# pixeru/bpm_analysis

Measured on AMD Instinct MI355X. Metric: audio-samples/sec (filter+envelope+peaks), 1024x60s@44.1kHz batch, 1 & 8 GPU, higher is better.
Workload: dtype f64; 1 GPU; 1024 x 60 s 44100 Hz mono int16 recordings per GPU, native mode (filter+envelope+noise floor+raw peaks); mode=native, parallelism=file-sharded x1, batch_pipeline=False

## Files before the change

bpm_analysis_amd/_native.py:

```python
from __future__ import annotations

import ctypes
import os

_HERE = os.path.dirname(os.path.abspath(__file__))
LIB_PATH = os.environ.get("BPMX_LIB") or os.path.join(_HERE, "libbpmx.so")

ABI_VERSION = 2

DT_U8, DT_I16, DT_I32, DT_F32, DT_F64 = 0, 1, 2, 3, 4
MODE_REFERENCE, MODE_NATIVE = 0, 1
STAGE_ENVELOPE, STAGE_FLOOR, STAGE_PEAKS, STAGE_ALL = 1, 2, 4, 7
F_STATIC_FLOOR, F_DRAFT_FLOOR, F_NAN_FLOOR, F_TOO_SHORT, F_BAD_WINDOW = 1, 2, 4, 8, 16
F_TROUGH_TIE, F_PEAK_TIE = 32, 64
F_TROUGH_ORDERED, F_PEAK_ORDERED = 128, 256
OPT_ROLLQ_MERGE = 1
OPT_NATIVE_F64 = 2
OPT_HILBERT_ROCFFT = 4
OPT_DRAFT_FULL = 8
OPT_ROLLQ_NOPRUNE = 16
OPT_DRAFT_GLOBAL_RANK = 32
OPT_ROLLQ_GLOBAL = 64
OPT_NATIVE_DMA = 128
OPT_PEAKS_GLOBAL = 256
OPT_HILBERT_R2C = 512
OPT_REF_SERIAL_MEAN = 1024
OPT_STATS = 2048
OPT_HILBERT_BLUESTEIN = 4096
OPT_REF_NOSPLIT = 8192
STAT_RAW_TROUGHS, STAT_UNDECIDED, STAT_FULL_DRAFT, NSTATS = 0, 1, 2, 8
OK, E_ARG, E_HIP, E_LIMIT, E_NODEV = 0, -1, -2, -3, -4

EXPORTS = ["bpmx_abi_version", "bpmx_last_error", "bpmx_create", "bpmx_destroy", "bpmx_decimated_length",
           "bpmx_run", "bpmx_run_ordered", "bpmx_synth", "bpmx_synth_host", "bpmx_profile", "bpmx_profile_read", "bpmx_profile_only",
           "bpmx_stats", "bpmx_set_pipeline"]


class Params(ctypes.Structure):
    _fields_ = [("mode", ctypes.c_int32), ("stages", ctypes.c_int32), ("dtype", ctypes.c_int32),
                ("channels", ctypes.c_int32), ("fs", ctypes.c_int32), ("ds", ctypes.c_int32),
                ("sr", ctypes.c_int32), ("env_window", ctypes.c_int32), ("distance", ctypes.c_int32),
                ("noise_window", ctypes.c_int32), ("min_periods", ctypes.c_int32), ("options", ctypes.c_int32),
                ("trough_prom_q", ctypes.c_double), ("peak_prom_q", ctypes.c_double),
                ("noise_floor_q", ctypes.c_double), ("fallback_q", ctypes.c_double),
                ("reject_mult", ctypes.c_double),
                ("ba_b", ctypes.c_double * 5), ("ba_a", ctypes.c_double * 5), ("ba_zi", ctypes.c_double * 4),
                ("sos", ctypes.c_double * 12), ("sos_zi", ctypes.c_double * 4)]


class Batch(ctypes.Structure):
    _fields_ = [("n_files", ctypes.c_int32), ("reserved", ctypes.c_int32), ("pcm", ctypes.c_void_p),
                ("frame_offsets", ctypes.POINTER(ctypes.c_int64))]


class Out(ctypes.Structure):
    _fields_ = [("env", ctypes.c_void_p), ("floor", ctypes.c_void_p), ("y", ctypes.c_void_p),
                ("troughs", ctypes.c_void_p), ("peaks", ctypes.c_void_p), ("n_troughs", ctypes.c_void_p),
                ("n_peaks", ctypes.c_void_p), ("flags", ctypes.c_void_p), ("n_raw_troughs", ctypes.c_void_p)]


class PeakOrder(ctypes.Structure):
    _fields_ = [("cand", ctypes.c_void_p * 2), ("n_cand", ctypes.c_void_p * 2),
                ("rank", ctypes.c_void_p * 2), ("use_rank", ctypes.c_void_p * 2)]


class BpmxError(RuntimeError):

    def __init__(self, msg: str = "", code: int = None):
        super().__init__(msg)
        self.code = code

    @property
    def per_file(self) -> bool:
        return self.code in (E_ARG, E_LIMIT)


class BpmxArgError(BpmxError, ValueError):
    """BPMX_E_ARG: an argument the reference's own calls reject with ValueError
    (scipy find_peaks' distance check, pandas' rolling-window checks); the
    message is the library's, which repeats the reference-side wording."""


_lib = None
# ... 51 lines not shown
```

bpm_analysis_amd/csrc/bpmx_api.hip:

```cpp
#include <hip/hip_runtime.h>

#include <algorithm>
#include <climits>
#include <cstdio>
#include <cstring>
#include <cstdlib>
#include <map>
#include <mutex>
#include <string>
#include <vector>

#include "bpmx_common.h"
#include "bpmx_kernels.h"
#include "bpmx_ctx.h"
#include "bpmx_native.h"
#include "bpmx_fpscan.h"
#include "bpmx_synth.h"

#include <rocprofiler-sdk-roctx/roctx.h>

using namespace bpmx;

namespace bpmx {
thread_local std::string g_err;
// ... 623 lines not shown
        }
        if (bad_window)
            LAUNCH(ctx, s, "k_flag_window", k_flag_window, dim3((F + 255) / 256), dim3(256), 0, s, F, d_run1,
                   (int32_t *)O->flags);
        const bool floor_wm = !(P->options & (BPMX_OPT_ROLLQ_MERGE | BPMX_OPT_ROLLQ_GLOBAL | BPMX_OPT_ROLLQ_NOPRUNE)) &&
                              maxnd <= WM_MMAX;
        if (noise_lazy && !floor_wm) {
            QuantArgs a;
            a.env = O->env; a.doff = d_doff; a.active = d_active; a.n_files = F; a.qv = qv; a.skip_le = QR_MAX;
            a.n_levels = 1; a.q[0] = P->noise_floor_q; a.slot[0] = 1 << Q_NOISE;
            a.skip = d_run1; a.stats = 0;
            LAUNCH(ctx, s, "k_quantile_reg", k_quantile_reg, dim3(F), dim3(QR_T), 0, s, a, bs);
        }
        const int64_t W = bad_window ? P->min_periods : P->noise_window;
        const int cap = (int)((W + RQ_T - 1 + 63) / 64 * 64);
        const size_t lds = rollq_lds_bytes(RQ_T, cap);
        const bool use_wm = !(P->options & (BPMX_OPT_ROLLQ_MERGE | BPMX_OPT_ROLLQ_GLOBAL));
        const bool need_merge = !use_wm || maxnd > WM_MMAX;
        const bool merge_g = need_merge && (cap > 32 * RQ_T || W + RQ_T >= 65000 || (P->options & BPMX_OPT_ROLLQ_GLOBAL));
        const int64_t gcap = (std::min<int64_t>(W + RQ_T, maxnd + 64) + 63) / 64 * 64;
        const size_t lds_g = rollq_g_lds_bytes(RQ_T, gcap);
        if (merge_g && lds_g > 160 * 1024)
            return fail(BPMX_E_LIMIT, "noise window and recording both longer than " +
                                          std::to_string((160 * 1024 - 16384) / 4 * 64) + " samples");
        uint16_t *wm_pos = use_wm ? (uint16_t *)ctx->buf("wm_pos", (size_t)sumnd * 2, &rc) : nullptr;
        int32_t *wm_full = use_wm ? (int32_t *)ctx->buf("wm_full", (size_t)F * 4, &rc) : nullptr;
        if (rc != BPMX_OK) return rc;
        const int64_t wm_n = std::min<int64_t>(maxnd, WM_MMAX);
        const size_t wm_lds_p = wm_layout(wm_n, true).total, wm_lds = wm_layout(wm_n, false).total;
        const int64_t wm_c = (WM_MMAX - W + 1) / 64 * 64;
        const bool wm_chunks = use_wm && maxnd > WM_MMAX && !(P->options & BPMX_OPT_ROLLQ_NOPRUNE) && wm_c >= 2048;
        const int64_t wm_nch = wm_chunks ? (maxnd + wm_c - 1) / wm_c : 1;
        int32_t *wm_fail = wm_chunks ? (int32_t *)ctx->buf("wm_fail", (size_t)F * 4, &rc) : nullptr;
        uint16_t *wm_pos_ch = wm_chunks ? (uint16_t *)ctx->buf("wm_pos_ch", (size_t)F * wm_nch * WM_PMAX * 2, &rc) : nullptr;
        if (rc != BPMX_OK) return rc;
        if (wm_nch > 65535) return fail(BPMX_E_LIMIT, "recording too long for the chunked rolling quantile");
        const dim3 g2((unsigned)std::min<int64_t>((maxnd + 255) / 256, std::max<int64_t>(8, 2048 / F)), F);
        auto interp = [&](const int32_t *run, const int64_t *tr, const int32_t *ntr, int64_t skip_gt) -> int {
            InterpArgs a;
            a.env = O->env; a.doff = d_doff; a.troughs = tr; a.ntr = ntr; a.run = run; a.n_files = F;
            a.dense = dense; a.skip_n = use_wm ? WM_MMAX : -1; a.skip_gt = skip_gt;
            const dim3 gi = maxnd <= WM_MMAX && use_wm ? dim3(2, (unsigned)F) : g2;
            LAUNCH(ctx, s, "k_interp", k_interp, gi, dim3(256), 0, s, a);
            return BPMX_OK;
        };
        auto rollq = [&](const int32_t *run, const int64_t *tr, const int32_t *ntr, double *outp,
                         int32_t *allnan, const double *tv) -> int {
            RollqArgs a;
            a.dense = dense; a.doff = d_doff; a.troughs = tr; a.tv = tv; a.run = run; a.n_files = F;
            a.env = O->env; a.ntr = ntr;
            a.window = (int32_t)W; a.min_periods = P->min_periods; a.cap = cap; a.q = P->noise_floor_q;
            a.out = outp; a.allnan = allnan; a.wm_max = use_wm ? WM_MMAX : 0;
            a.wm_chunk = 0; a.wm_fail = wm_fail; a.wm_pos_ch = wm_pos_ch;
            int rq_rc = BPMX_OK;
            int32_t *vfl = need_merge ? (int32_t *)ctx->buf("rollq_valid", (size_t)F * 8, &rq_rc) : nullptr;
            if (rq_rc != BPMX_OK) return rq_rc;
            a.vfirst = vfl;
            a.vlast = vfl ? vfl + F : nullptr;
            if (need_merge) {
                HIP_TRY(hipMemsetAsync(a.vfirst, 0x7F, (size_t)F * 4, s));
                HIP_TRY(hipMemsetAsync(a.vlast, 0xFF, (size_t)F * 4, s));
            }
            if (wm_chunks) {
                HIP_TRY(hipMemsetAsync(wm_fail, 0, (size_t)F * 4, s));
                a.wm_chunk = (int32_t)wm_c;
            }
            if (need_merge && (rq_rc = interp(run, tr, ntr, wm_chunks ? WM_MMAX : INT64_MAX)) != BPMX_OK) return rq_rc;
            if (use_wm) {
                wm_lds_attr(ctx->device);
                if (!(P->options & BPMX_OPT_ROLLQ_NOPRUNE))
                    LAUNCH(ctx, s, "k_rollq_wm", k_rollq_wm_t<true>, dim3(F, (unsigned)wm_nch), dim3(WM_T),
                           std::max(wm_lds_p, wm_lds), s, a, wm_pos, wm_full);
                else
                    LAUNCH(ctx, s, "k_rollq_wm[full]", k_rollq_wm_t<false>, dim3(F), dim3(WM_T), wm_lds, s, a, wm_pos,
                           wm_full);
            }
            if (!need_merge) return BPMX_OK;
            RollqArgs fill = a;
            if (wm_chunks) {
                a.run = wm_fail;
                if ((rq_rc = interp(wm_fail, tr, ntr, INT64_MAX)) != BPMX_OK) return rq_rc;
            }
            a.chunk = 8192;
            while (a.chunk > 1024 && (int64_t)F * ((maxnd + a.chunk - 1) / a.chunk) < 1024) a.chunk >>= 1;
            if (merge_g) a.chunk = std::max<int64_t>(a.chunk, (W + RQ_T - 1) / RQ_T * RQ_T);
            const int64_t nch = (maxnd + a.chunk - 1) / a.chunk;
            if (nch > 65535) return fail(BPMX_E_LIMIT, "recording too long for the chunked rolling quantile");
            const dim3 gq((unsigned)F, (unsigned)nch);
            if (merge_g) {
                a.gcap = gcap;
                a.gv = (double *)ctx->buf("rollq_gv", (size_t)F * nch * 2 * gcap * 8, &rq_rc);
                a.gp = (int32_t *)ctx->buf("rollq_gp", (size_t)F * nch * 2 * gcap * 4, &rq_rc);
                if (rq_rc != BPMX_OK) return rq_rc;
                (void)hipFuncSetAttribute((const void *)k_rolling_quantile_g<RQ_T>,
                                          hipFuncAttributeMaxDynamicSharedMemorySize, (int)lds_g);
                LAUNCH(ctx, s, "k_rolling_quantile", (k_rolling_quantile_g<RQ_T>), gq, dim3(RQ_T), lds_g, s, a);
            } else if (cap <= 16 * RQ_T) {
                (void)hipFuncSetAttribute((const void *)k_rolling_quantile<RQ_T, 16>,
                                          hipFuncAttributeMaxDynamicSharedMemorySize, (int)lds);
                LAUNCH(ctx, s, "k_rolling_quantile", (k_rolling_quantile<RQ_T, 16>), gq, dim3(RQ_T), lds, s, a);
            } else {
                (void)hipFuncSetAttribute((const void *)k_rolling_quantile<RQ_T, 32>,
                                          hipFuncAttributeMaxDynamicSharedMemorySize, (int)lds);
                LAUNCH(ctx, s, "k_rolling_quantile", (k_rolling_quantile<RQ_T, 32>), gq, dim3(RQ_T), lds, s, a);
            }
            LAUNCH(ctx, s, "k_rollq_fill", k_rollq_fill, dim3(4, (unsigned)F), dim3(256), 0, s, fill);
            return BPMX_OK;
        };
        uint8_t *tdec = nullptr;
        int32_t *d_exact = d_run1, *d_runfb = nullptr;
        if (bounds) {
            tdec = (uint8_t *)ctx->buf("trough_dec", (size_t)sumnd, &rc);
            if (rc != BPMX_OK) return rc;
            d_exact = draft_masks;
            d_runfb = draft_masks + F;
            DraftBoundArgs a;
            a.env = O->env; a.doff = d_doff; a.raw = rawt; a.rawv = rawv; a.nraw = d_nraw; a.run = d_run1;
            a.n_files = F;
            a.window = (int32_t)W; a.min_periods = P->min_periods; a.q = P->noise_floor_q; a.mult = P->reject_mult;
            a.dec = tdec; a.exact = d_exact;
            a.local_m = (P->options & BPMX_OPT_DRAFT_GLOBAL_RANK) ? INT_MAX : DB_LOCAL_M;
            a.stats = d_stats;
            if (rc != BPMX_OK) return rc;
            const int64_t trmax = maxnd / std::max<int64_t>(1, P->distance) + 1;
            const unsigned gy = (unsigned)std::max<int64_t>(1, (trmax + DB_T - 1) / DB_T);
            a.vfl = draft_vfl;
            a.nund = draft_vfl + 2 * F;
            LAUNCH(ctx, s, "k_draft_bounds", k_draft_bounds, dim3(F, gy), dim3(DB_T), 0, s, a);
#ifndef BPMX_DP_GY
#define BPMX_DP_GY 4
#endif
            const unsigned gp = (unsigned)std::max<int64_t>(1, std::min<int64_t>(BPMX_DP_GY, (trmax + DP_CHUNK - 1) / DP_CHUNK));
            LAUNCH(ctx, s, "k_draft_points", k_draft_points<1>, dim3(F, gp), dim3(DB_T), 0, s, a);
            LAUNCH(ctx, s, "k_draft_points[wide]", k_draft_points<4>, dim3(F, gp), dim3(DB_T), 0, s, a);
        }
        SanitizeArgs sa;
        sa.env = O->env; sa.draft = draft; sa.doff = d_doff; sa.active = d_active; sa.raw = rawt; sa.nraw = d_nraw;
        sa.rawv = rawv; sa.outv = trv;
        sa.n_files = F; sa.mult = P->reject_mult; sa.out = O->troughs; sa.nout = O->n_troughs; sa.flags = O->flags;
        sa.run2 = d_run2; sa.dec = tdec; sa.exact = d_exact; sa.run_fb = d_runfb;
        if (floor_wm) {
            FloorWmArgs a;
            a.rq.dense = dense; a.rq.doff = d_doff; a.rq.n_files = F; a.rq.env = O->env;
            a.rq.window = (int32_t)W; a.rq.min_periods = P->min_periods; a.rq.cap = cap; a.rq.q = P->noise_floor_q;
            a.rq.wm_max = WM_MMAX; a.rq.wm_chunk = 0; a.rq.wm_fail = nullptr; a.rq.wm_pos_ch = nullptr;
            a.rq.vfirst = a.rq.vlast = nullptr; a.rq.chunk = 0; a.rq.gv = nullptr; a.rq.gp = nullptr; a.rq.gcap = 0;
            a.rq.troughs = nullptr; a.rq.tv = nullptr; a.rq.ntr = nullptr; a.rq.run = nullptr; a.rq.out = nullptr;
            a.rq.allnan = nullptr;
#ifdef BPMX_STAMPS
            a.rq.stamps = nullptr;
#endif
            sa.run2 = nullptr; sa.run_fb = nullptr;
            a.sa = sa;
            a.exact = d_exact;
            a.qv = qv;
            a.qn = QuantArgs{};
            if (noise_lazy) {
                a.qn.env = O->env; a.qn.doff = d_doff; a.qn.active = d_active; a.qn.n_files = F; a.qn.qv = qv;
                a.qn.skip_le = QR_MAX; a.qn.n_levels = 1; a.qn.q[0] = P->noise_floor_q; a.qn.slot[0] = 1 << Q_NOISE;
                a.qn.skip = nullptr; a.qn.stats = 0;
            }
            a.floor = O->floor; a.draft = draft; a.an_draft = d_an1; a.an_final = d_an2; a.full = wm_full;
            if ((rc = rollq(d_exact, rawt, d_nraw, draft, d_an1, rawv)) != BPMX_OK) return rc;
            wm_lds_attr(ctx->device);
            LAUNCH(ctx, s, "k_floor_wm", k_floor_wm, dim3(F), dim3(WM_T), std::max(wm_lds_p, wm_lds), s, a);
        }
        if (!floor_wm && (rc = rollq(d_exact, rawt, d_nraw, draft, d_an1, rawv)) != BPMX_OK) return rc;
        if (!floor_wm) {
            SanitizeArgs a;
            a.env = O->env; a.draft = draft; a.doff = d_doff; a.active = d_active; a.raw = rawt; a.nraw = d_nraw;
            a.rawv = rawv; a.outv = trv;
            a.n_files = F; a.mult = P->reject_mult; a.out = O->troughs; a.nout = O->n_troughs; a.flags = O->flags;
            a.run2 = d_run2; a.dec = tdec; a.exact = d_exact; a.run_fb = d_runfb;
            LAUNCH(ctx, s, "k_sanitize", k_sanitize, dim3(F), dim3(256), 0, s, a);
        }
        if (!floor_wm && bounds && (rc = rollq(d_runfb, rawt, d_nraw, draft, d_an1, rawv)) != BPMX_OK) return rc;
        if (!floor_wm && (rc = rollq(d_run2, O->troughs, O->n_troughs, O->floor, d_an2, trv)) != BPMX_OK) return rc;
        if (!floor_wm) {
            FinalArgs a;
            a.draft = draft; a.doff = d_doff; a.active = d_active; a.qv = qv; a.allnan_draft = d_an1;
            a.allnan_final = d_an2; a.n_files = F; a.floor = O->floor; a.flags = O->flags;
#ifndef BPMX_FF_WIDE
            const dim3 gf(maxnd > 65536 ? g2.x : 1u, (unsigned)F);
#else
            const dim3 gf = g2;
#endif
            LAUNCH(ctx, s, "k_floor_final", k_floor_final, gf, dim3(256), 0, s, a);
        }
    }

    if (do_peaks) {
        StageRange range("bpmx:peaks");
        PeakArgs a;
        a.env = O->env; a.height = O->floor; a.doff = d_doff; a.boff = d_boff; a.active = d_active;
        a.bmax = bmax; a.bmin = bmin; a.qv = qv; a.qslot = Q_PEAK; a.n_files = F; a.distance = P->distance;
        a.sign = 1.0; a.cand = cand; a.state = state; a.out = O->peaks; a.nout = O->n_peaks;
        a.run_out = nullptr; a.run_min = 0; a.tie_bit = BPMX_F_PEAK_TIE;
        a.scan_ok = fp_scan; a.scan_cnt = fp_scan + F;
        set_order(a, 1);
        FIND_PEAKS(a, "peaks");
    }
// ... 161 lines not shown
```

bpm_analysis_amd/csrc/bpmx_kernels.h:

```cpp
#ifndef BPMX_KERNELS_H
#define BPMX_KERNELS_H

#include "bpmx_common.h"

namespace bpmx {

enum { Q_TROUGH = 0, Q_PEAK = 1, Q_NOISE = 2, Q_FALLBACK = 3, Q_SLOTS = 4 };

struct InitOutArgs {
    const int32_t *active;
    int32_t *flags, *ntr, *npk, *runs, *nraw;
    int32_t *z1;
    int32_t *z2;
    int32_t *z3;
    int32_t n_files;
};
__device__ __forceinline__ void init_out_one(const InitOutArgs &I, int f) {
    const int F = I.n_files;
    I.flags[f] = I.active[f] ? 0 : BPMX_F_TOO_SHORT;
    if (I.ntr) I.ntr[f] = 0;
    if (I.npk) I.npk[f] = 0;
    for (int k = 0; k < 5; ++k) I.runs[(int64_t)k * F + f] = 0;
    if (I.nraw) I.nraw[f] = 0;
    if (I.z1) I.z1[f] = 0;
// ... 159 lines not shown
    int32_t *mtot;
    int32_t *mp;
    double *mh;
    double *vv;
    double *b32h, *b32l, *b32r;
    double *b1kh, *b1kl, *b1kr;
    int32_t *dfail;
    int32_t dchunk;
};
constexpr int FPC_T = 256, FPC_S = 1024, FPC_H = 1024, FPC_R = (FPC_S + FPC_H) / FPC_T;
__host__ __device__ inline int64_t fpl_b32_off(int64_t d0, int f) { return (d0 >> 5) + 4 * (int64_t)f; }
__host__ __device__ inline int64_t fpl_b1k_off(int64_t d0, int f) { return (d0 >> 10) + 4 * (int64_t)f; }
__global__ void k_fpl_scan(PeakArgs A, FplArgs L);
__global__ void k_fpl_place(PeakArgs A, FplArgs L);
__global__ void k_fpl_fill(PeakArgs A, FplArgs L);
__global__ void k_fpl_distance(PeakArgs A, FplArgs L);
__global__ void k_fpl_dist_ch(PeakArgs A, FplArgs L);
__global__ void k_fpl_prom(PeakArgs A, FplArgs L);
__global__ void k_fpl_compact(PeakArgs A, FplArgs L);

struct InterpArgs {
    const double *env;
    const int64_t *doff;
    const int64_t *troughs;
    const int32_t *ntr;
    const int32_t *run;
    int32_t n_files;
    double *dense;
    int64_t skip_n;
    int64_t skip_gt;
};

struct RollqArgs {
    const double *dense;
    const int64_t *doff;
    const int64_t *troughs;
    const int32_t *run;
    int32_t n_files, window, min_periods, cap;
    double q;
    double *out;
    int32_t *allnan;
    int32_t wm_max;
    const double *env;
    const double *tv;
    const int32_t *ntr;
    int64_t chunk;
    int32_t *vfirst, *vlast;
    double *gv;
    int32_t *gp;
    int64_t gcap;
    int32_t wm_chunk;
    int32_t *wm_fail;
    uint16_t *wm_pos_ch;
#ifdef BPMX_STAMPS
    unsigned long long *stamps;
#endif
};

struct SanitizeArgs {
    const double *env, *draft;
    const int64_t *doff;
    const int32_t *active;
    const int64_t *raw;
    const double *rawv;
    const int32_t *nraw;
    int32_t n_files;
    double mult;
    double *outv;
    int64_t *out;
    int32_t *nout;
    int32_t *flags;
    int32_t *run2;
    const uint8_t *dec;
    const int32_t *exact;
    int32_t *run_fb;
};

template <int NT>
__device__ __forceinline__ int sanitize_wg(const SanitizeArgs &A, int f, int *sh) {
    const int64_t d0 = A.doff[f];
    const int64_t *raw = A.raw + d0;
    int64_t *out = A.out + d0;
    const int m = A.nraw[f];
    const int tid = threadIdx.x;
    const double *rawv = A.rawv + d0;
    double *outv = A.outv + d0;
    if (m < 5) {
        for (int j = tid; j < m; j += NT) { out[j] = raw[j]; outv[j] = rawv[j]; }
        if (tid == 0) {
            A.nout[f] = m;
            A.flags[f] |= BPMX_F_STATIC_FLOOR;
            if (A.run2) A.run2[f] = 0;
        }
        return m;
    }
    const double *draft = A.draft + d0;
    const bool exact = !A.dec || A.exact[f];
    int w = 0;
    for (int c0 = 0; c0 < m; c0 += NT) {
        const int j = c0 + tid;
        bool keep = false;
        int64_t t = 0;
        double tv = 0.0;
        if (j < m) {
            t = raw[j];
            tv = rawv[j];
// ... 51 lines not shown
constexpr int DB_LOCAL_M = 512;
struct DbSeg {
    int32_t s, e;
    double v;
};

struct FinalArgs {
    const double *draft;
    const int64_t *doff;
    const int32_t *active;
    const double *qv;
    const int32_t *allnan_draft, *allnan_final;
    int32_t n_files;
    double *floor;
    int32_t *flags;
};

__host__ __device__ inline size_t rollq_lds_bytes(int T, int cap) {
    return (size_t)cap * 10 + (size_t)T * 20 + ((size_t)T + 1) * 4 + ((size_t)T / 64 + 2) * 4;
}
constexpr int RQ_T = 256;

template <int DT, bool MULTI, bool ZB>
__global__ void k_envelope_ref_t(EnvRefArgs A);
template <int DT, bool MULTI>
__global__ void k_ref_pick(EnvRefArgs A);
__global__ void k_quantile_reg(QuantArgs A, BlockStatArgs B);
__global__ void k_block_stats(BlockStatArgs A);
__global__ void k_find_peaks(PeakArgs A);
__global__ void k_find_peaks_lds(PeakArgs A);
__global__ void k_interp(InterpArgs A);
__global__ void k_sanitize(SanitizeArgs A);
__global__ void k_draft_bounds(DraftBoundArgs A);
template <int SPL>
__global__ void k_draft_points(DraftBoundArgs A);
__global__ void k_floor_final(FinalArgs A);
template <int T, int RQ_MAXCH>
__global__ void k_rolling_quantile(RollqArgs A);
template <int T>
__global__ void k_rolling_quantile_g(RollqArgs A);
__host__ __device__ inline size_t rollq_g_lds_bytes(int T, int64_t gcap) {
    return (size_t)T * 16 + (size_t)T * 8 + ((size_t)T + 1) * 4 + ((size_t)T / 64 + 2) * 4 + (size_t)T * 16 +
           ((size_t)(gcap / 64) + 2) * 4;
}
__global__ void k_rollq_fill(RollqArgs A);

constexpr int WM_T = 1024;
constexpr int WM_ITEMS = 18;
constexpr int WM_MMAX = WM_T * WM_ITEMS;
constexpr int WM_TRMAX = 512;
constexpr int WM_PMAX = 12288;
constexpr int WM_DCAP = 96;
constexpr int WM_WSCR = WM_DCAP;
struct WmLayout {
    size_t tab, meta, kpos, area, total;
};
constexpr int WM_NBK = WM_MMAX / 64 + 2;
constexpr int WM_META_LOW = (WM_NBK * 22 + 7) & ~7;
constexpr int WM_META_B = WM_META_LOW + WM_NBK * 22;
__host__ __device__ inline size_t wm_align16(size_t x) { return (x + 15) & ~(size_t)15; }
__host__ __device__ inline WmLayout wm_layout(int64_t nmax, bool prune) {
    const int64_t n = nmax < 1 ? 1 : (nmax > WM_MMAX ? WM_MMAX : nmax);
    const int64_t m = prune && n > WM_PMAX ? WM_PMAX : n;
    const int64_t L = m > 1 ? 64 - __builtin_clzll((unsigned long long)(m - 1)) : 1;
    const int64_t NW = (m + 63) / 64;
    const int64_t m8 = (m + 7) & ~7LL;
    const int64_t NBK = WM_MMAX / 64 + 2;
    const int64_t sort_b = 8 * m8 + (int64_t)(WM_T / 64) * 128 * 4;
    const int64_t wm_b = ((4 * m8 + 15) & ~15LL) + (int64_t)(WM_T / 64) * WM_WSCR * 4;
    (void)L; (void)NW;
    const int64_t hist_b = prune ? NBK * 64 * 2 + (int64_t)(WM_T / 64) * 64 * 4 + n : 0;
    int64_t area = sort_b > wm_b ? sort_b : wm_b;
    area = area > hist_b ? area : hist_b;
    WmLayout l;
    l.tab = 0;
    l.meta = wm_align16((size_t)WM_TRMAX * (prune ? 20 : 12) + (size_t)NBK * 4);
    l.kpos = wm_align16(l.meta + (prune ? (size_t)WM_META_B : 0));
    l.area = wm_align16(l.kpos + (prune ? (size_t)m * 2 : 0));
    l.total = l.area + (size_t)area;
    return l;
}
template <bool PRUNE>
__global__ void k_rollq_wm_t(RollqArgs A, uint16_t *pos_scratch, int32_t *full);
__global__ void k_floor_wm(FloorWmArgs A);

}

#endif
```

bpm_analysis_amd/csrc/k_rollq_wm.hip:

```cpp
#include "bpmx_common.h"
#include "bpmx_kernels.h"
#include "bpmx_stamps.h"
#include "bpmx_qsel.h"

namespace bpmx {

__device__ __forceinline__ uint64_t wm_key(double v) {
    return f64_key(v == 0.0 ? 0.0 : v);
}

__device__ __forceinline__ uint64_t lanemask_lt() {
    return (1ull << lane_id()) - 1ull;
}

__device__ __forceinline__ uint64_t match8(uint32_t dg) {
    uint64_t m = ~0ull;
#pragma unroll
    for (int b = 0; b < 8; ++b) {
        const uint64_t bal = __ballot((dg >> b) & 1u);
        m &= ((dg >> b) & 1u) ? bal : ~bal;
    }
    return m;
}

struct RqShared {
    int jlo, jhi, first, last, wt[WM_T / 64], mk;
    unsigned long long orv[WM_T / 64], andv[WM_T / 64];
    double vmin, vmax;
};

template <bool PRUNE>
__device__ __forceinline__ bool rollq_wm_body(RollqArgs A, uint16_t *pos_scratch, int32_t *full, RqShared &S_) {
    constexpr int NWV = WM_T / 64;
    constexpr int MMAX = PRUNE ? WM_PMAX : WM_MMAX;
    constexpr int MAXIT = MMAX / WM_T;
    const int f = blockIdx.x;
    if (f >= A.n_files) return false;
    const int tid = threadIdx.x, lane = lane_id(), wid = wave_id();
    if (!A.run[f]) {
        if (PRUNE && tid == 0) full[f] = 0;
        return false;
    }
    const int64_t d0 = A.doff[f], n = A.doff[f + 1] - d0;
    const int ntr_all = A.env ? A.ntr[f] : 0;
    const bool chunked = PRUNE && A.wm_chunk > 0 && n > WM_MMAX && A.env;
    if (!chunked && blockIdx.y > 0) return false;
    const int64_t W = A.window, minp = A.min_periods;
    int64_t o0 = 0, o1 = n, t0 = 0, top = n;
    int jlo = 0, ntr = ntr_all;
    int &s_jlo = S_.jlo, &s_jhi = S_.jhi;
    if (chunked) {
        if (tid == 0 && blockIdx.y == 0) full[f] = 0;
        o0 = (int64_t)blockIdx.y * A.wm_chunk;
        if (o0 >= n) return false;
        o1 = min<int64_t>(n, o0 + A.wm_chunk);
        int64_t s, e;
        win_bounds(o0, n, W, s, e);
        const int64_t *tr = A.troughs + d0;
// ... 269 lines not shown
                    const int y = __shfl_up(x, o);
                    if (lane >= o) x += y;
                }
                if (pb < NPB) pre[pb] = run + x - v;
                run += __shfl(x, 63);
            }
            if (lane == 0) {
                pre[NPB] = run;
                if (!wid) s_mk = run;
            }
        }
        __syncthreads();
        kc = s_mk;
        STAMP(13);
        if (kc > WM_PMAX) {
            if (tid == 0) { if (chunked) A.wm_fail[f] = 1; else full[f] = 1; }
            return !chunked;
        }
        if (tid == 0 && !chunked) full[f] = 0;
        for (int pb = wid; pb < NPB; pb += NWV) {
            const uint64_t mk = kmask[pb];
            if ((mk >> lane) & 1) kpos[kpre[pb] + __popcll(mk & lanemask_lt())] = (uint16_t)((pb << 6) + lane);
        }
        m = kc;
        __syncthreads();
    }
#ifdef RQ_STOP_PRUNE
    return false;
#endif
    auto spos = [&](int c) -> int { return PRUNE ? (int)kpos[c] : c; };
    auto kidx = [&](int p) -> int {
        if (!PRUNE) return p;
        const uint64_t mk = kmask[p >> 6];
        return kpre[p >> 6] + __popcll(mk & ((1ull << (p & 63)) - 1ull));
    };
    auto lidx = [&](int p) -> int {
        const uint64_t mk = lmask[p >> 6];
        return lpre[p >> 6] + __popcll(mk & ((1ull << (p & 63)) - 1ull));
    };
    STAMP(7);
#ifdef RQ_DIAG_M
    if (threadIdx.x == 0) _st_acc[13] = (unsigned long long)m;
#endif

    const int IT = (m + WM_T - 1) / WM_T;
    const int mu = __builtin_amdgcn_readfirstlane(m), ITu = __builtin_amdgcn_readfirstlane(IT);
    const int S = 64 * IT;
    const int m8 = (m + 7) & ~7;
    uint16_t *posA = (uint16_t *)(smem + Lay.area);
    uint16_t *posB = posA + m8;
    uint32_t *kh = (uint32_t *)(posB + m8);
    uint32_t *cnt = kh + m8;
    const size_t wbin_off = (size_t)8 * m8 + (size_t)NWV * 128 * 4;
    unsigned long long *wbin_all =
        wbin_off + (size_t)NWV * 256 * 8 <= Lay.total - Lay.area ? (unsigned long long *)(smem + Lay.area + wbin_off) : nullptr;

    const size_t wsc = ((size_t)4 * m8 + 15) & ~(size_t)15;
    const size_t svl_off = wsc + (size_t)NWV * WM_WSCR * 4;
    double *svl = svl_off + (size_t)8 * m <= Lay.total - Lay.area ? (double *)(smem + Lay.area + svl_off) : nullptr;
    uint64_t kbase = 0;
    int shc = 0;
    if (PRUNE && svl) {
        kbase = wm_key(s_vmin);
        const uint64_t ktop = wm_key(s_vmax);
        const int nbits = ktop > kbase ? 64 - __clzll((long long)(ktop - kbase)) : 0;
        shc = nbits > 40 ? nbits - 40 : 0;
    }
    {
        auto ckey = [&](int p) -> uint64_t {
            const uint64_t k = wm_key(dval(t0 + spos(p)));
            return shc ? (k > kbase ? k - kbase : 0ull) >> shc : k;
        };
        uint64_t kor = 0, kand = ~0ull;
        for (int p = tid; p < m; p += WM_T) {
            posA[p] = (uint16_t)p;
            const uint64_t k = ckey(p);
            kh[p] = (uint32_t)k;
            kor |= k;
            kand &= k;
        }
        for (int o = 32; o > 0; o >>= 1) {
            kor |= (uint64_t)__shfl_xor((long long)kor, o);
            kand &= (uint64_t)__shfl_xor((long long)kand, o);
        }
        if (lane == 0) { s_or[wid] = kor; s_and[wid] = kand; }
        if (wbin_all)
            for (int j = tid; j < NWV * 256; j += WM_T) wbin_all[j] = 0ull;
        __syncthreads();
        uint64_t vary = 0;
        {
            uint64_t o = 0, a = ~0ull;
            for (int w = 0; w < NWV; ++w) { o |= s_or[w]; a &= s_and[w]; }
            vary = o ^ a;
        }
        STAMP(0);
        uint32_t *wc = cnt + wid * 128;
        for (int d = 0; d < 8; ++d) {
            if (d == 4 && (vary >> 32)) {
                for (int p = tid; p < m; p += WM_T) kh[p] = (uint32_t)(ckey(p) >> 32);
                __syncthreads();
            }
            if (((vary >> (8 * d)) & 0xFFull) == 0) continue;
            const int sh = 8 * (d & 3);
            for (int j = lane; j < 128; j += 64) wc[j] = 0;
            uint32_t dg8[(MAXIT + 3) / 4], rk16[(MAXIT + 1) / 2];
            int mo = mu, ITo = ITu, sb = wid * S + lane;
            asm volatile("" : "+s"(mo), "+s"(ITo), "+v"(sb));
#pragma unroll
            for (int i = 0; i < MAXIT; ++i) {
                const int slot = sb + i * 64;
                const uint32_t dg = (i < ITo && slot < mo) ? (kh[posA[slot]] >> sh) & 0xFFu : 0u;
                if ((i & 3) == 0) dg8[i >> 2] = dg; else dg8[i >> 2] |= dg << (8 * (i & 3));
            }
            __builtin_amdgcn_wave_barrier();
            asm volatile("" : "+s"(mo), "+s"(ITo), "+v"(sb));
#pragma unroll
            for (int i = 0; i < MAXIT; ++i) {
                if (i < ITo) {
                    const int slot = sb + i * 64;
                    const bool valid = slot < mo;
                    const uint32_t dg = (dg8[i >> 2] >> (8 * (i & 3))) & 0xFFu;
                    uint64_t peers;
                    if (wbin_all) {
                        unsigned long long *bin = wbin_all + wid * 256 + dg;
                        if (valid) atomicOr(bin, 1ull << lane);
                        peers = __hip_atomic_load(bin, __ATOMIC_RELAXED, __HIP_MEMORY_SCOPE_WORKGROUP);
                    } else {
                        peers = match8(dg);
                    }
                    peers &= __ballot(valid);
                    const uint64_t below = peers & lanemask_lt();
                    const int leader = valid ? __ffsll((long long)peers) - 1 : lane;
                    uint32_t base = 0;
                    if (valid && below == 0) {
                        base = atomicAdd(&wc[dg >> 1], (uint32_t)__popcll(peers) << (16 * (dg & 1)));
                        if (wbin_all) __hip_atomic_store(wbin_all + wid * 256 + dg, 0ull, __ATOMIC_RELAXED,
                                                         __HIP_MEMORY_SCOPE_WORKGROUP);
                    }
                    base = (uint32_t)__shfl((int)base, leader);
                    const uint32_t rnk = ((base >> (16 * (dg & 1))) & 0xFFFFu) + (uint32_t)__popcll(below);
                    if ((i & 1) == 0) rk16[i >> 1] = rnk; else rk16[i >> 1] |= rnk << 16;
                }
            }
            __syncthreads();
            STAMP(1);
            {
                uint32_t v[4], sm = 0;
#pragma unroll
                for (int u = 0; u < 4; ++u) {
                    const int e = tid * 4 + u, dg = e / NWV, w = e % NWV;
                    v[u] = (cnt[w * 128 + (dg >> 1)] >> (16 * (dg & 1))) & 0xFFFFu;
                    sm += v[u];
                }
                uint32_t x = sm;
                for (int o = 1; o < 64; o <<= 1) {
                    const uint32_t y = __shfl_up(x, o);
                    if (lane >= o) x += y;
                }
                if (lane == 63) s_wt[wid] = (int)x;
                __syncthreads();
                uint32_t run = x - sm;
                for (int w = 0; w < wid; ++w) run += (uint32_t)s_wt[w];
                uint16_t *c16 = (uint16_t *)cnt;
#pragma unroll
                for (int u = 0; u < 4; ++u) {
                    const int e = tid * 4 + u, dg = e / NWV, w = e % NWV;
                    c16[(w * 128 + (dg >> 1)) * 2 + (dg & 1)] = (uint16_t)run;
                    run += v[u];
                }
            }
            __syncthreads();
            STAMP(2);
            const uint16_t *c16 = (const uint16_t *)cnt;
            asm volatile("" : "+s"(mo), "+s"(ITo), "+v"(sb));
#pragma unroll
            for (int i = 0; i < MAXIT; ++i) {
                const int slot = sb + i * 64;
                if (i < ITo && slot < mo) {
                    const uint32_t dg = (dg8[i >> 2] >> (8 * (i & 3))) & 0xFFu;
                    const uint32_t rnk = (rk16[i >> 1] >> (16 * (i & 1))) & 0xFFFFu;
                    posB[(int)c16[(wid * 128 + (dg >> 1)) * 2 + (dg & 1)] + (int)rnk] = posA[slot];
                }
            }
            __syncthreads();
            uint16_t *t = posA; posA = posB; posB = t;
            STAMP(3);
        }
    }
    uint16_t *posR = posA, *rkx = posB;
    for (int r = tid; r < m; r += WM_T) rkx[posR[r]] = (uint16_t)r;
    if (svl)
        for (int r = tid; r < m; r += WM_T) svl[r] = dval(t0 + spos(posR[r]));
    __syncthreads();
    if (shc) {
        bool down = false;
        for (int r = tid; r + 1 < m; r += WM_T) down |= svl[r] > svl[r + 1];
        if (__syncthreads_or(down)) {
            if (tid == 0) { if (chunked) A.wm_fail[f] = 1; else full[f] = 1; }
            return !chunked;
        }
    }
#ifdef RQ_STOP_SORT
    return false;
#endif
    uint32_t *wl = (uint32_t *)(smem + Lay.area + wsc) + (size_t)wid * WM_WSCR;
    STAMP(5);

    auto target = [&](int nb, double &idxf, bool &interp) -> int {
        idxf = 0;
        int k = 0;
        if (nb > 1) {
            idxf = q * (double)(nb - 1);
            k = (int)idxf;
        }
        interp = !(nb == 1 || (double)k == idxf);
        return k;
    };
    const uint64_t ltm = lanemask_lt();
    const int off = (int)((W - 1) / 2), Wi = (int)W, ni = (int)n, t0i = (int)t0;
#ifdef RQ_DIAG_Q
    unsigned long long dq[8] = {0};
#endif
    int vfirst = INT_MAX, vlast = -1;
#ifdef RQ_DIAG_W
    const unsigned long long tw0 = __builtin_amdgcn_s_memtime();
#endif
    {
        const int NBLK = (int)((o1 - o0 + 63) >> 6);
        const int NBW = (NBLK + NWV - 1) / NWV;
        const int b0 = wid * NBW, b1 = min(NBLK, b0 + NBW);
        int rs = 0, cU = 0, pPlo = -1, pPhi = -1;
        for (int bk = b0; bk < b1; ++bk) {
            const int i0 = (int)o0 + (bk << 6), i = i0 + lane;
            bool valid = false;
            int plo = 0, phi = 0, t = 0, nobs = 0, kq = 0;
            double idxq = 0.0;
            bool intq = false;
            if (i < (int)o1) {
                const int ee = i + 1 + off, ss = ee - Wi;
                const int e = ee < ni ? ee : ni, sc = ss > 0 ? ss : 0;
                const int lo = sc > t0i ? sc : t0i;
                nobs = e > lo ? e - lo : 0;
                if (nobs >= minp && nobs > 0) {
                    valid = true;
                    plo = kidx(lo - t0i);
                    phi = kidx(e - t0i);
                    const int lw = PRUNE ? lidx(e - t0i) - lidx(lo - t0i) : 0;
// ... 291 lines not shown
```

bpm_analysis_amd/engine.py:

```python
from __future__ import annotations

import ctypes
import threading
from dataclasses import dataclass
from typing import List, Optional, Sequence

import numpy as np

from . import _native as N
from .design import Design, design, detect_design, dtype_code, make_params

MODES = {"reference": N.MODE_REFERENCE, "native": N.MODE_NATIVE}


def _torch():
    import torch
    return torch


_TORCH_DT = None


def torch_dtype(np_dtype):
    global _TORCH_DT
# ... 222 lines not shown
        ev = torch.cuda.Event()
        ev.record(torch.cuda.current_stream(self.device))
        return host, ev

    def tie_check_finish(self, handle, out: Result, params: dict, stages: int = N.STAGE_ALL,
                         options: int = 0) -> int:
        host, ev = handle
        ev.synchronize()
        bits = N.F_TROUGH_TIE | N.F_PEAK_TIE
        if not (host.numpy() & bits).any():
            return 0
        return self.resolve_ties(out, params, stages, options)

    def synth(self, frame_offsets: Sequence[int], fs: int, channels: int = 1, seed0: int = 0,
              seeds: Optional[Sequence[int]] = None):
        torch = _torch()
        fo = np.ascontiguousarray(frame_offsets, dtype=np.int64)
        pcm = torch.empty(int(fo[-1]) * channels, dtype=torch.int16, device=self.device)
        runs = [(seed0, 0, len(fo) - 1)] if seeds is None else [(int(sd), f, f + 1) for f, sd in enumerate(seeds)]
        with self.lock:
            for sd, a, b in runs:
                sub = np.ascontiguousarray(fo[a:b + 1])
                N.check(self.L.bpmx_synth(self.ctx, sd, b - a, sub.ctypes.data_as(ctypes.POINTER(ctypes.c_int64)),
                                          fs, channels, ctypes.c_void_p(pcm.data_ptr()), self.stream_handle()),
                        "bpmx_synth")
        return pcm

    def profile(self, on: bool):
        N.check(self.L.bpmx_profile(self.ctx, 1 if on else 0), "bpmx_profile")

    def profile_only(self, label: str = ""):
        N.check(self.L.bpmx_profile_only(self.ctx, label.encode()), "bpmx_profile_only")

    def profile_read(self) -> dict:
        buf = ctypes.create_string_buffer(1 << 16)
        n = self.L.bpmx_profile_read(self.ctx, buf, len(buf))
        if n < 0:
            N.check(n, "bpmx_profile_read")
        out = {}
        for line in buf.value.decode().splitlines():
            name, cnt, ms = line.rsplit(" ", 2)
            out[name] = (int(cnt), float(ms))
        return out

    def set_pipeline(self, chunks: int, env_cus: int = 0, det_cus: int = 0):
        N.check(self.L.bpmx_set_pipeline(self.ctx, chunks, env_cus, det_cus), "bpmx_set_pipeline")

    def stats(self) -> dict:
        buf = (ctypes.c_int64 * N.NSTATS)()
        rc = self.L.bpmx_stats(self.ctx, buf, N.NSTATS)
        if rc < 0:
            N.check(rc, "bpmx_stats")
        return {"raw_troughs": int(buf[N.STAT_RAW_TROUGHS]), "undecided": int(buf[N.STAT_UNDECIDED]),
                "full_draft_chunks": int(buf[N.STAT_FULL_DRAFT])}

    def run_host(self, recordings: List[np.ndarray], fs: int, params: dict, mode: str = "reference",
                 stages: int = N.STAGE_ALL, want_y: bool = False, log: bool = False,
                 options: int = 0, longest_first: bool = True, resolve_ties: bool = False) -> List[dict]:
        torch = _torch()
        if not recordings:
            return []
        if longest_first and len({r.shape[0] for r in recordings}) > 1:
            from .shard import longest_first as _lf
            perm = _lf([r.shape[0] for r in recordings])
            res = self.run_host([recordings[i] for i in perm], fs, params, mode=mode, stages=stages,
                                want_y=want_y, log=log, options=options, longest_first=False,
                                resolve_ties=resolve_ties)
            out: List[dict] = [None] * len(recordings)
            for k, i in enumerate(perm):
                out[i] = res[k]
            return out
        dt = recordings[0].dtype
        ch = 1 if recordings[0].ndim == 1 else recordings[0].shape[1]
        for r in recordings:
            if r.dtype != dt or (1 if r.ndim == 1 else r.shape[1]) != ch:
                raise ValueError("a batch needs one sample format and channel count")
        fo = np.zeros(len(recordings) + 1, dtype=np.int64)
        fo[1:] = np.cumsum([r.shape[0] for r in recordings])
        host = np.concatenate([np.ascontiguousarray(r).reshape(-1) for r in recordings])
        with self.lock, torch.cuda.stream(self.host_stream()):
            pcm = torch.from_numpy(host).to(self.device)
            res = self.run(pcm, fo, fs, params, mode=mode, stages=stages, channels=ch, want_y=want_y, log=log,
                           options=options)
            if resolve_ties:
                self.resolve_ties(res, params, stages, options)
            out = res.to_host()
            self.host_stream().synchronize()
        return out

    def run_env_host(self, envs: List[np.ndarray], sr: int, params: dict, stages: int,
                     floors: Optional[List[np.ndarray]] = None, options: int = 0,
                     resolve_ties: bool = False) -> List[dict]:
        torch = _torch()
        fo = np.zeros(len(envs) + 1, dtype=np.int64)
        fo[1:] = np.cumsum([len(e) for e in envs])
        d = detect_design(sr, params)
        with self.lock, torch.cuda.stream(self.host_stream()):
            out = self.alloc(fo, 1, d.sr)
            out.env.copy_(torch.from_numpy(np.concatenate(envs).astype(np.float64)).to(self.device))
            if floors is not None:
                out.floor.copy_(torch.from_numpy(np.concatenate(floors).astype(np.float64)).to(self.device))
            self.run(None, fo, d.sr, params, stages=stages, out=out, d=d, options=options)
            if resolve_ties:
                self.resolve_ties(out, params, stages, options)
            res = out.to_host()
            self.host_stream().synchronize()
        return res
# ... 127 lines not shown
```

include/bpmx.h:

```cpp
#ifndef BPMX_H
#define BPMX_H

#include <stdint.h>

#ifdef __cplusplus
extern "C" {
#endif

#define BPMX_ABI_VERSION 2

enum bpmx_dtype { BPMX_DT_U8 = 0, BPMX_DT_I16 = 1, BPMX_DT_I32 = 2, BPMX_DT_F32 = 3, BPMX_DT_F64 = 4 };

enum bpmx_mode { BPMX_MODE_REFERENCE = 0, BPMX_MODE_NATIVE = 1 };

enum bpmx_stage {
    BPMX_STAGE_ENVELOPE = 1,
    BPMX_STAGE_FLOOR = 2,
    BPMX_STAGE_PEAKS = 4,
    BPMX_STAGE_ALL = 7
};

enum bpmx_status {
    BPMX_OK = 0,
    BPMX_E_ARG = -1,
    BPMX_E_HIP = -2,
    BPMX_E_LIMIT = -3,
    BPMX_E_NODEV = -4
};

enum bpmx_file_flag {
    BPMX_F_STATIC_FLOOR = 1,
    BPMX_F_DRAFT_FLOOR = 2,
    BPMX_F_NAN_FLOOR = 4,
    BPMX_F_TOO_SHORT = 8,
    BPMX_F_BAD_WINDOW = 16,
    BPMX_F_TROUGH_TIE = 32,
    BPMX_F_PEAK_TIE = 64,
    BPMX_F_TROUGH_ORDERED = 128,
    BPMX_F_PEAK_ORDERED = 256
};

enum bpmx_option {
    BPMX_OPT_ROLLQ_MERGE = 1,
    BPMX_OPT_NATIVE_F64 = 2,
    BPMX_OPT_HILBERT_ROCFFT = 4,
    BPMX_OPT_DRAFT_FULL = 8,
    BPMX_OPT_ROLLQ_NOPRUNE = 16,
    BPMX_OPT_DRAFT_GLOBAL_RANK = 32,
    BPMX_OPT_ROLLQ_GLOBAL = 64,
    BPMX_OPT_NATIVE_DMA = 128,
    BPMX_OPT_PEAKS_GLOBAL = 256,
    BPMX_OPT_HILBERT_R2C = 512,
    BPMX_OPT_REF_SERIAL_MEAN = 1024,
    BPMX_OPT_STATS = 2048,
    BPMX_OPT_HILBERT_BLUESTEIN = 4096,
    BPMX_OPT_REF_NOSPLIT = 8192
};

enum bpmx_stat {
    BPMX_STAT_RAW_TROUGHS = 0,
    BPMX_STAT_UNDECIDED = 1,
    BPMX_STAT_FULL_DRAFT = 2,
    BPMX_NSTATS = 8
};

typedef struct bpmx_ctx bpmx_ctx;

typedef struct {
    int32_t mode;
    int32_t stages;
    int32_t dtype;
    int32_t channels;
    int32_t fs;
    int32_t ds;
    int32_t sr;
    int32_t env_window;
    int32_t distance;
    int32_t noise_window;
    int32_t min_periods;
    int32_t options;
    double trough_prom_q;
    double peak_prom_q;
    double noise_floor_q;
    double fallback_q;
    double reject_mult;
    double ba_b[5], ba_a[5], ba_zi[4];
    double sos[12], sos_zi[4];
} bpmx_params;

typedef struct {
    int32_t n_files;
    int32_t reserved;
    const void *pcm;
    const int64_t *frame_offsets;
} bpmx_batch;

typedef struct {
    double *env;
    double *floor;
    double *y;
    int64_t *troughs;
    int64_t *peaks;
    int32_t *n_troughs;
    int32_t *n_peaks;
    int32_t *flags;
    int32_t *n_raw_troughs;
} bpmx_out;

int bpmx_abi_version(void);
const char *bpmx_last_error(void);

int bpmx_create(int device, bpmx_ctx **out);
void bpmx_destroy(bpmx_ctx *ctx);

int64_t bpmx_decimated_length(int64_t n_frames, int32_t ds);
// ... 32 lines not shown
```

Measured before the change: 1190 billion audio-samples/s.

## Rank short rolling-quantile windows by a 24-bit key prefix plus tie-cell fixup

For short windows in the pruned wavelet-matrix rolling quantile, the values are cached in shared memory and keys are range-normalised to a 24-bit prefix. The radix sort then stops after the prefix digits, and the groups of equal prefixes are finished with small wave-level rank sorts. This is meant to skip the remaining radix passes and the repeated global value gathers. If any group is too large, the block falls back to the full sort. An option forces the full sort, and new counters record how often each path is taken.

```diff
diff --git a/bpm_analysis_amd/_native.py b/bpm_analysis_amd/_native.py
--- a/bpm_analysis_amd/_native.py
+++ b/bpm_analysis_amd/_native.py
@@ -28,7 +28,9 @@
 OPT_STATS = 2048
 OPT_HILBERT_BLUESTEIN = 4096
 OPT_REF_NOSPLIT = 8192
+OPT_ROLLQ_FULLSORT = 16384
 STAT_RAW_TROUGHS, STAT_UNDECIDED, STAT_FULL_DRAFT, NSTATS = 0, 1, 2, 8
+STAT_RANK_SHORT, STAT_RANK_RESORT = 3, 4
 OK, E_ARG, E_HIP, E_LIMIT, E_NODEV = 0, -1, -2, -3, -4
 
 EXPORTS = ["bpmx_abi_version", "bpmx_last_error", "bpmx_create", "bpmx_destroy", "bpmx_decimated_length",
diff --git a/bpm_analysis_amd/csrc/bpmx_api.hip b/bpm_analysis_amd/csrc/bpmx_api.hip
--- a/bpm_analysis_amd/csrc/bpmx_api.hip
+++ b/bpm_analysis_amd/csrc/bpmx_api.hip
@@ -699,6 +699,7 @@
             a.window = (int32_t)W; a.min_periods = P->min_periods; a.cap = cap; a.q = P->noise_floor_q;
             a.out = outp; a.allnan = allnan; a.wm_max = use_wm ? WM_MMAX : 0;
             a.wm_chunk = 0; a.wm_fail = wm_fail; a.wm_pos_ch = wm_pos_ch;
+            a.stats = d_stats; a.rank_full = (P->options & BPMX_OPT_ROLLQ_FULLSORT) ? 1 : 0;
             int rq_rc = BPMX_OK;
             int32_t *vfl = need_merge ? (int32_t *)ctx->buf("rollq_valid", (size_t)F * 8, &rq_rc) : nullptr;
             if (rq_rc != BPMX_OK) return rq_rc;
@@ -794,6 +795,7 @@
             a.rq.vfirst = a.rq.vlast = nullptr; a.rq.chunk = 0; a.rq.gv = nullptr; a.rq.gp = nullptr; a.rq.gcap = 0;
             a.rq.troughs = nullptr; a.rq.tv = nullptr; a.rq.ntr = nullptr; a.rq.run = nullptr; a.rq.out = nullptr;
             a.rq.allnan = nullptr;
+            a.rq.stats = d_stats; a.rq.rank_full = (P->options & BPMX_OPT_ROLLQ_FULLSORT) ? 1 : 0;
 #ifdef BPMX_STAMPS
             a.rq.stamps = nullptr;
 #endif
diff --git a/bpm_analysis_amd/csrc/bpmx_kernels.h b/bpm_analysis_amd/csrc/bpmx_kernels.h
--- a/bpm_analysis_amd/csrc/bpmx_kernels.h
+++ b/bpm_analysis_amd/csrc/bpmx_kernels.h
@@ -235,6 +235,8 @@
     int32_t wm_chunk;
     int32_t *wm_fail;
     uint16_t *wm_pos_ch;
+    int64_t *stats;
+    int32_t rank_full;
 #ifdef BPMX_STAMPS
     unsigned long long *stamps;
 #endif
@@ -392,6 +394,8 @@
 constexpr int WM_PMAX = 12288;
 constexpr int WM_DCAP = 96;
 constexpr int WM_WSCR = WM_DCAP;
+constexpr int WM_CELL_CAP = 32;
+constexpr int WM_SP_IT = 7;
 struct WmLayout {
     size_t tab, meta, kpos, area, total;
 };
diff --git a/bpm_analysis_amd/csrc/k_rollq_wm.hip b/bpm_analysis_amd/csrc/k_rollq_wm.hip
--- a/bpm_analysis_amd/csrc/k_rollq_wm.hip
+++ b/bpm_analysis_amd/csrc/k_rollq_wm.hip
@@ -4,6 +4,12 @@
 #include "bpmx_qsel.h"
 
 namespace bpmx {
+
+#ifndef RQ_PREFIX_BITS
+#define RQ_PREFIX_BITS 24
+#endif
+constexpr int WM_PFX_BITS = RQ_PREFIX_BITS;
+static_assert(WM_PFX_BITS >= 8 && WM_PFX_BITS <= 24 && WM_PFX_BITS % 8 == 0, "whole 8-bit digits of the low key half");
 
 __device__ __forceinline__ uint64_t wm_key(double v) {
     return f64_key(v == 0.0 ? 0.0 : v);
@@ -379,8 +385,7 @@
     uint32_t *kh = (uint32_t *)(posB + m8);
     uint32_t *cnt = kh + m8;
     const size_t wbin_off = (size_t)8 * m8 + (size_t)NWV * 128 * 4;
-    unsigned long long *wbin_all =
-        wbin_off + (size_t)NWV * 256 * 8 <= Lay.total - Lay.area ? (unsigned long long *)(smem + Lay.area + wbin_off) : nullptr;
+    bool use_bins = wbin_off + (size_t)NWV * 256 * 8 <= Lay.total - Lay.area;
 
     const size_t wsc = ((size_t)4 * m8 + 15) & ~(size_t)15;
     const size_t svl_off = wsc + (size_t)NWV * WM_WSCR * 4;
@@ -393,36 +398,158 @@
         const int nbits = ktop > kbase ? 64 - __clzll((long long)(ktop - kbase)) : 0;
         shc = nbits > 40 ? nbits - 40 : 0;
     }
+    bool shortp = false;
+    size_t val_off = 0;
+    if (PRUNE && svl && !A.rank_full && m <= WM_SP_IT * WM_T) {
+        const size_t room = Lay.total - Lay.area, with_bins = wm_align16(wbin_off + (size_t)NWV * 256 * 8);
+        if (with_bins + (size_t)8 * m <= room) {
+            shortp = true;
+            val_off = with_bins;
+        } else if (wm_align16(wbin_off) + (size_t)8 * m <= room) {
+            shortp = true;
+            use_bins = false;
+            val_off = wm_align16(wbin_off);
+        }
+    }
+    const bool useval = shortp;
+    double *const val = (double *)(smem + Lay.area + val_off);
+    unsigned long long *const wbin_all = use_bins ? (unsigned long long *)(smem + Lay.area + wbin_off) : nullptr;
     {
         auto ckey = [&](int p) -> uint64_t {
-            const uint64_t k = wm_key(dval(t0 + spos(p)));
+            const uint64_t k = wm_key(PRUNE && useval ? val[p] : dval(t0 + spos(p)));
             return shc ? (k > kbase ? k - kbase : 0ull) >> shc : k;
         };
-        uint64_t kor = 0, kand = ~0ull;
-        for (int p = tid; p < m; p += WM_T) {
-            posA[p] = (uint16_t)p;
-            const uint64_t k = ckey(p);
-            kh[p] = (uint32_t)k;
-            kor |= k;
-            kand &= k;
-        }
-        for (int o = 32; o > 0; o >>= 1) {
-            kor |= (uint64_t)__shfl_xor((long long)kor, o);
-            kand &= (uint64_t)__shfl_xor((long long)kand, o);
-        }
-        if (lane == 0) { s_or[wid] = kor; s_and[wid] = kand; }
-        if (wbin_all)
-            for (int j = tid; j < NWV * 256; j += WM_T) wbin_all[j] = 0ull;
-        __syncthreads();
         uint64_t vary = 0;
-        {
+        auto init_full = [&]() {
+            uint64_t kor = 0, kand = ~0ull;
+            for (int p = tid; p < m; p += WM_T) {
+                posA[p] = (uint16_t)p;
+                const uint64_t k = ckey(p);
+                kh[p] = (uint32_t)k;
+                kor |= k;
+                kand &= k;
+            }
+            for (int o = 32; o > 0; o >>= 1) {
+                kor |= (uint64_t)__shfl_xor((long long)kor, o);
+                kand &= (uint64_t)__shfl_xor((long long)kand, o);
+            }
+            if (lane == 0) { s_or[wid] = kor; s_and[wid] = kand; }
+            __syncthreads();
             uint64_t o = 0, a = ~0ull;
             for (int w = 0; w < NWV; ++w) { o |= s_or[w]; a &= s_and[w]; }
             vary = o ^ a;
+        };
+        if (wbin_all)
+            for (int j = tid; j < NWV * 256; j += WM_T) wbin_all[j] = 0ull;
+        if (PRUNE && shortp) {
+            uint64_t kmn = ~0ull, kmx = 0ull;
+            for (int p = tid; p < m; p += WM_T) {
+                posA[p] = (uint16_t)p;
+                const double v = dval(t0 + spos(p));
+                val[p] = v;
+                const uint64_t k = wm_key(v);
+                kmn = k < kmn ? k : kmn;
+                kmx = k > kmx ? k : kmx;
+            }
+            for (int o = 32; o > 0; o >>= 1) {
+                const uint64_t a = (uint64_t)__shfl_xor((long long)kmn, o), b = (uint64_t)__shfl_xor((long long)kmx, o);
+                kmn = a < kmn ? a : kmn;
+                kmx = b > kmx ? b : kmx;
+            }
+            if (lane == 0) { s_or[wid] = kmx; s_and[wid] = kmn; }
+            __syncthreads();
+            for (int w = 0; w < NWV; ++w) {
+                kmx = s_or[w] > kmx ? s_or[w] : kmx;
+                kmn = s_and[w] < kmn ? s_and[w] : kmn;
+            }
+            const uint64_t span = kmx > kmn ? kmx - kmn : 0ull;
+            const int nbits = span ? 64 - __clzll((long long)span) : 0;
+            const int psh = nbits > WM_PFX_BITS ? nbits - WM_PFX_BITS : 0;
+            vary = span >> psh;
+            for (int b = 1; b < WM_PFX_BITS; b <<= 1) vary |= vary >> b;
+            for (int p = tid; p < m; p += WM_T) kh[p] = (uint32_t)((wm_key(val[p]) - kmn) >> psh);
+            __syncthreads();
+        } else {
+            init_full();
         }
         STAMP(0);
         uint32_t *wc = cnt + wid * 128;
         for (int d = 0; d < 8; ++d) {
+            if (PRUNE && shortp && d == WM_PFX_BITS / 8) {
+                static_assert(WM_CELL_CAP <= 32, "a half wave per side");
+                uint32_t *cells = wc;
+                int ncw = 0;
+                bool over = false;
+                for (int i = 0; i < ITu; ++i) {
+                    const int rb = wid * S + i * 64, r = rb + lane;
+                    bool mark = false;
+                    uint32_t px = 0;
+                    uint64_t kl = 0;
+                    if (r > 0 && r < m) {
+                        const int x = posA[r], xl = posA[r - 1];
+                        px = kh[x];
+                        if (px == kh[xl]) {
+                            kl = wm_key(val[xl]);
+                            mark = wm_key(val[x]) != kl;
+                        }
+                    }
+                    uint64_t fm = __ballot(mark);
+                    while (fm) {
+                        const int l0 = __ffsll((long long)fm) - 1, r0 = rb + l0;
+                        const uint32_t pxu = (uint32_t)__builtin_amdgcn_readlane((int)px, l0);
+                        const uint64_t klu = ((uint64_t)(uint32_t)__builtin_amdgcn_readlane((int)(kl >> 32), l0) << 32) |
+                                             (uint32_t)__builtin_amdgcn_readlane((int)kl, l0);
+                        const int rr = lane < 32 ? r0 - 1 - lane : r0 + lane - 32;
+                        bool same = false, eqk = false;
+                        if (rr >= 0 && rr < m) {
+                            const int y = posA[rr];
+                            same = kh[y] == pxu;
+                            eqk = same && wm_key(val[y]) == klu;
+                        }
+                        const uint64_t sm = __ballot(same), em = __ballot(eqk);
+                        const uint32_t sl = (uint32_t)sm, sr = (uint32_t)(sm >> 32), el = (uint32_t)em;
+                        const int ll = sl == ~0u ? 32 : __ffs((int)~sl) - 1;
+                        const int rl = sr == ~0u ? 32 : __ffs((int)~sr) - 1;
+                        const uint32_t lm = ll >= 32 ? ~0u : (1u << ll) - 1u;
+                        if ((~el & lm) != 0u) {
+                            fm &= fm - 1;
+                            continue;
+                        }
+                        if (ll + rl > WM_CELL_CAP || ncw >= 128) {
+                            over = true;
+                        } else {
+                            if (lane == 0) cells[ncw] = (uint32_t)(r0 - ll) | ((uint32_t)(ll + rl) << 16);
+                            ++ncw;
+                        }
+                        const int hl = l0 + rl;
+                        fm &= hl >= 64 ? 0ull : ~((1ull << hl) - 1ull);
+                    }
+                }
+                over = __syncthreads_or(over) != 0;
+                if (A.stats && tid == 0)
+                    atomicAdd((unsigned long long *)&A.stats[over ? BPMX_STAT_RANK_RESORT : BPMX_STAT_RANK_SHORT], 1ull);
+                if (!over) {
+                    for (int c = 0; c < ncw; ++c) {
+                        const uint32_t ce = (uint32_t)__builtin_amdgcn_readfirstlane((int)cells[c]);
+                        const int lo = (int)(ce & 0xFFFFu), len = min(min((int)(ce >> 16), WM_CELL_CAP), m - lo);
+                        const bool in = lane < len;
+                        const int e = in ? (int)posA[lo + lane] : 0;
+                        const uint64_t k = in ? wm_key(val[e]) : 0ull;
+                        int rk = 0;
+                        for (int j = 0; j < len; ++j) {
+                            const uint64_t kj = ((uint64_t)(uint32_t)__builtin_amdgcn_readlane((int)(k >> 32), j) << 32) |
+                                                (uint32_t)__builtin_amdgcn_readlane((int)k, j);
+                            rk += (kj < k || (kj == k && j < lane)) ? 1 : 0;
+                        }
+                        if (in) posA[lo + rk] = (uint16_t)e;
+                    }
+                    __syncthreads();
+                    break;
+                }
+                shortp = false;
+                init_full();
+                d = 0;
+            }
             if (d == 4 && (vary >> 32)) {
                 for (int p = tid; p < m; p += WM_T) kh[p] = (uint32_t)(ckey(p) >> 32);
                 __syncthreads();
@@ -515,11 +642,32 @@
         }
     }
     uint16_t *posR = posA, *rkx = posB;
-    for (int r = tid; r < m; r += WM_T) rkx[posR[r]] = (uint16_t)r;
-    if (svl)
-        for (int r = tid; r < m; r += WM_T) svl[r] = dval(t0 + spos(posR[r]));
+    if (PRUNE && useval) {
+        svl = val;
+        double gv[WM_SP_IT];
+#pragma unroll
+        for (int i = 0; i < WM_SP_IT; ++i) {
+            const int r = tid + i * WM_T;
+            gv[i] = 0.0;
+            if (r < m) {
+                const int x = posR[r];
+                rkx[x] = (uint16_t)r;
+                gv[i] = val[x];
+            }
+        }
+        __syncthreads();
+#pragma unroll
+        for (int i = 0; i < WM_SP_IT; ++i) {
+            const int r = tid + i * WM_T;
+            if (r < m) svl[r] = gv[i];
+        }
+    } else {
+        for (int r = tid; r < m; r += WM_T) rkx[posR[r]] = (uint16_t)r;
+        if (svl)
+            for (int r = tid; r < m; r += WM_T) svl[r] = dval(t0 + spos(posR[r]));
+    }
     __syncthreads();
-    if (shc) {
+    if (shc || (PRUNE && useval)) {
         bool down = false;
         for (int r = tid; r + 1 < m; r += WM_T) down |= svl[r] > svl[r + 1];
         if (__syncthreads_or(down)) {
diff --git a/bpm_analysis_amd/engine.py b/bpm_analysis_amd/engine.py
--- a/bpm_analysis_amd/engine.py
+++ b/bpm_analysis_amd/engine.py
@@ -298,7 +298,8 @@
         if rc < 0:
             N.check(rc, "bpmx_stats")
         return {"raw_troughs": int(buf[N.STAT_RAW_TROUGHS]), "undecided": int(buf[N.STAT_UNDECIDED]),
-                "full_draft_chunks": int(buf[N.STAT_FULL_DRAFT])}
+                "full_draft_chunks": int(buf[N.STAT_FULL_DRAFT]),
+                "rank_short": int(buf[N.STAT_RANK_SHORT]), "rank_resort": int(buf[N.STAT_RANK_RESORT])}
 
     def run_host(self, recordings: List[np.ndarray], fs: int, params: dict, mode: str = "reference",
                  stages: int = N.STAGE_ALL, want_y: bool = False, log: bool = False,
diff --git a/include/bpmx.h b/include/bpmx.h
--- a/include/bpmx.h
+++ b/include/bpmx.h
@@ -54,13 +54,16 @@
     BPMX_OPT_REF_SERIAL_MEAN = 1024,
     BPMX_OPT_STATS = 2048,
     BPMX_OPT_HILBERT_BLUESTEIN = 4096,
-    BPMX_OPT_REF_NOSPLIT = 8192
+    BPMX_OPT_REF_NOSPLIT = 8192,
+    BPMX_OPT_ROLLQ_FULLSORT = 16384
 };
 
 enum bpmx_stat {
     BPMX_STAT_RAW_TROUGHS = 0,
     BPMX_STAT_UNDECIDED = 1,
     BPMX_STAT_FULL_DRAFT = 2,
+    BPMX_STAT_RANK_SHORT = 3,
+    BPMX_STAT_RANK_RESORT = 4,
     BPMX_NSTATS = 8
 };
 
```

After: 1195 billion audio-samples/s, median of 3. Within noise of the previous version (+0.4%).
